# ToddThomson/Mila

Hardware: AMD Instinct MI355X
Metric: Gemma-4 12B decode tok/s (B=1, context 2048), 1xMI355X (higher is better)
Workload: dtype bf16; 1 GPU; Gemma-4 12B, weight policy bf16, B=1, prefill T=2048 then decode at positions 2048..; decode_mode=graph, replicas=1, parallelism=replicas only (no collective), bounded_local_kv=0

## Files before the change

mila_amd/csrc/attention.hip:

```cpp
#include "common.h"
#include "rms_common.h"
#include "rope_common.h"
#include "internal.h"
#include "attention_generic.h"
#include "attention_tiles.h"
#include "attention_decode_mfma.h"
#include "attention_decode_plan.h"
#include "attention_decode_scalar.h"

namespace mila {

__global__ __launch_bounds__(256) void kv_write_bf16_kernel(uint16_t* __restrict__ Kc, uint16_t* __restrict__ Vc,
                                                            const uint16_t* __restrict__ k,
                                                            const uint16_t* __restrict__ v, int64_t total_vec,
                                                            int chunk, int NKV, int HS, int start_pos, int capacity)
{
    const int hv = HS / 8;
    const int64_t stride = (int64_t)gridDim.x * 256;
    for (int64_t i = (int64_t)blockIdx.x * 256 + threadIdx.x; i < total_vec; i += stride)
    {
        const int e = (int)(i % hv);
        int64_t r = i / hv;
        const int n = (int)(r % NKV);
        r /= NKV;
        const int t = (int)(r % chunk);
        const int b = (int)(r / chunk);
        const int row = (start_pos + t) % capacity;
        const size_t dst = ((((size_t)b * NKV + n) * capacity + row) * hv + e) * 8;
        st16(Kc + dst, ld16(k + i * 8));
        st16(Vc + dst, ld16(v + i * 8));
    }
}

struct AttnParams
{
    uint16_t* Y;
    const uint16_t* Q;
    int64_t q_b_stride;
    uint16_t* K;
    uint16_t* V;
    float* scratch;
    int no_combine;
    const uint8_t* warm_a; int64_t warm_a_lines; int warm_a_blocks;
    const uint8_t* warm_b; int64_t warm_b_lines; int warm_b_blocks; int64_t warm_b_pair;
    uint32_t* tickets;
    int NH, NKV, capacity, position, window, splits;
    float scale;
    const int32_t* pos_dev;
    int flat;
    int64_t raw_b_stride;
    const uint16_t* q_raw;
    const uint16_t* k_raw;
    const uint16_t* v_raw;
    const uint16_t* qw;
    const uint16_t* kw;
    const uint16_t* vw;
    const float* cos_cache;
    const float* sin_cache;
    float eps;
    int pos_stride;
};

template <int HS>
__device__ __forceinline__ void head_row_post(const uint16_t* __restrict__ src, const uint16_t* __restrict__ w, bool rotate,
                                              const float* cos_row, const float* sin_row, float eps,
                                              uint16_t* dst_lds, uint16_t* dst_glb)
{
    constexpr int hv = HS / 16;
    const int lane = threadIdx.x & 63;
    const bool act = lane < hv;
    const int l2 = act ? lane : 0;
    const u32x4 xlo = ld16(src + (size_t)l2 * 8), xhi = ld16(src + (size_t)(l2 + hv) * 8);
    u32x4 wlo = u32x4{0u, 0u, 0u, 0u}, whi = wlo;
    if (w) { wlo = ld16(w + (size_t)l2 * 8); whi = ld16(w + (size_t)(l2 + hv) * 8); }
    const float rstd = rms_rstd_wave(src, HS, eps);
    if (act)
    {
        u32x4 lo, hi;
        if (w) { lo = rms_apply8(xlo, wlo, rstd, 0.0f); hi = rms_apply8(xhi, whi, rstd, 0.0f); }
        else { lo = rms_apply8_now(xlo, rstd); hi = rms_apply8_now(xhi, rstd); }
        if (rotate) rope_rotate8_vals(lo, hi, cos_row, sin_row, lane * 8);
        if (dst_lds) { st16(dst_lds + (size_t)lane * 8, lo); st16(dst_lds + (size_t)(lane + hv) * 8, hi); }
        if (dst_glb) { st16(dst_glb + (size_t)lane * 8, lo); st16(dst_glb + (size_t)(lane + hv) * 8, hi); }
    }
}

template <bool SC1>
__device__ __forceinline__ float partial_ld(const float* p)
{
    if constexpr (SC1)
        return __hip_atomic_load((const __attribute__((address_space(1))) float*)p, __ATOMIC_RELAXED, __HIP_MEMORY_SCOPE_AGENT);
    else
        return *p;
}
template <bool SC1>
__device__ __forceinline__ uint16_t combine_dim(const float* __restrict__ base, int HS, int splits, int d)
{
    const int STR = HS + 4;
    const int s = threadIdx.x & 63;
    float vals[16];
#pragma unroll
    for (int u = 0; u < 16; ++u) vals[u] = (u < splits) ? partial_ld<SC1>(base + (size_t)u * STR + d) : 0.0f;
    const float ms = (s < splits) ? partial_ld<SC1>(base + (size_t)s * STR + HS) : -INFINITY;
    const float ls = (s < splits) ? partial_ld<SC1>(base + (size_t)s * STR + HS + 1) : 0.0f;
    float acc = 0.0f;
    const float M = wave_max(ms);
    const float fs = (ms == -INFINITY) ? 0.0f : __expf(ms - M);
    const float L = wave_sum(ls * fs);
    const int n8 = (splits + 7) & ~7;
    for (int i0 = 0; i0 < n8; i0 += 16)
    {
        if (i0 > 0)
        {
#pragma unroll
            for (int u = 0; u < 16; ++u) vals[u] = (i0 + u < splits) ? partial_ld<SC1>(base + (size_t)(i0 + u) * STR + d) : 0.0f;
        }
#pragma unroll
        for (int u = 0; u < 16; ++u)
        {
            const float f = __uint_as_float(__builtin_amdgcn_readlane(__float_as_uint(fs), min(i0 + u, 63)));
            if (i0 + u < n8) acc = fmaf(vals[u], f, acc);
        }
    }
    return f32_to_bf16_bits(L > 0.0f ? acc / L : 0.0f);
}

__device__ __forceinline__ void warm_lines(const uint8_t* __restrict__ base, int64_t nlines, int64_t tid, int64_t nthreads, float* never,
                                           int64_t pair = 0)
{
    uint32_t acc = 0;
    int64_t i = tid;
    auto at = [&](int64_t l) { return pair ? base + (l & 1) * pair + (l >> 1) * 128 : base + l * 128; };
    for (; i + 7 * nthreads < nlines; i += 8 * nthreads)
    {
        uint32_t v[8];
#pragma unroll
        for (int u = 0; u < 8; ++u) v[u] = *reinterpret_cast<const uint32_t*>(at(i + u * nthreads));
#pragma unroll
        for (int u = 0; u < 8; ++u) acc ^= v[u];
    }
    for (; i < nlines; i += nthreads) acc ^= *reinterpret_cast<const uint32_t*>(at(i));
    if (acc == 0x12345679u && never != nullptr) never[0] = 1.0f;
}

#ifdef MILA_ATTN_STAMPS
__device__ unsigned long long g_attn_stamps[2];
#endif

#define MILA_ATTN_LEAD_PARAMS const int32_t* pos_dev, uint16_t* K, uint16_t* V, const uint16_t* q_raw, int NH, int NKV, int capacity, int window, int splits, int flat
#define MILA_ATTN_LEAD_ARGS(p) (p).pos_dev, (p).K, (p).V, (p).q_raw, (p).NH, (p).NKV, (p).capacity, (p).window, (p).splits, ((p).flat | ((p).pos_stride ? 2 : 0))
__device__ __forceinline__ AttnParams attn_params(MILA_ATTN_LEAD_PARAMS, const AttnParams& tail)
{
    AttnParams p = tail;
    p.pos_dev = pos_dev; p.K = K; p.V = V; p.q_raw = q_raw;
    p.NH = NH; p.NKV = NKV; p.capacity = capacity; p.window = window; p.splits = splits; p.flat = flat & 1; p.pos_stride = (flat >> 1) & 1;
    return p;
}

template <int HS, int GH, bool FUSED>
__global__ __launch_bounds__(kDecodeWaves * 64) void attn_decode_kernel(MILA_ATTN_LEAD_PARAMS, const AttnParams tail)
{
#ifdef MILA_ATTN_STAMPS
    const unsigned long long entry_ = __builtin_amdgcn_s_memtime();
#endif
    const AttnParams p = attn_params(pos_dev, K, V, q_raw, NH, NKV, capacity, window, splits, flat, tail);
    using Row = DecodeGeomBf16<HS>;
    constexpr int NW = kDecodeWaves, EPL = Row::EPL, NPAIR = Row::NPAIR, ACTIVE = Row::ACTIVE, PG = Row::PG, STR = HS + 2;
    extern __shared__ __attribute__((aligned(16))) unsigned char smem_raw[];
    float* sm = reinterpret_cast<float*>(smem_raw);
    uint16_t* qs = reinterpret_cast<uint16_t*>(smem_raw + (size_t)NW * GH * STR * sizeof(float));

    const int lane = threadIdx.x & 63, wave = threadIdx.x >> 6;
    const bool owner = lane < ACTIVE;
    const int GS = p.NH / p.NKV, hgroups = GS / GH;
    if (!p.flat && (int)blockIdx.x >= p.splits)
    {
        const int64_t wb = ((int64_t)(blockIdx.x - p.splits) * gridDim.y + blockIdx.y) * gridDim.z + blockIdx.z;
        warm_lines(p.warm_a, p.warm_a_lines, wb * (NW * 64) + threadIdx.x, (int64_t)p.warm_a_blocks * gridDim.y * gridDim.z * (NW * 64),
                   p.scratch);
        return;
    }
    const int ngrp = p.NKV * hgroups;
    const int split = p.flat ? (int)blockIdx.x / ngrp : (int)blockIdx.x, grp = p.flat ? (int)blockIdx.x % ngrp : (int)blockIdx.y;
    const int kvh = grp / hgroups, hg = grp % hgroups;
    const int h0 = kvh * GS + hg * GH;
    const int b = blockIdx.z;
    const int pos = p.pos_dev ? p.pos_dev[b * p.pos_stride] : p.position;
    const int len = pos + 1;
    const int band_begin = (p.window > 0) ? max(0, len - p.window) : 0;
    const int band = len - band_begin;
    const int chunk = (band + p.splits - 1) / p.splits;
    const int begin = band_begin + split * chunk;
    const int end = min(begin + chunk, len);
    const bool owns_new = FUSED && pos >= begin && pos < end;

    uint16_t* kbase = p.K + ((size_t)b * p.NKV + kvh) * p.capacity * HS;
    uint16_t* vbase = p.V + ((size_t)b * p.NKV + kvh) * p.capacity * HS;

    struct KVG { uint32_t k[PG][NPAIR], v[PG][NPAIR]; };
    auto load_group = [&](KVG& gbuf, int base) {
#pragma unroll
        for (int j = 0; j < PG; ++j)
        {
            const int pp = base + NW * j;
            if (owner && pp < end && !(FUSED && pp == pos))
            {
                const size_t r = (size_t)(pp % p.capacity) * HS + lane * EPL;
                load_row<EPL>(gbuf.k[j], kbase + r);
                load_row<EPL>(gbuf.v[j], vbase + r);
            }
            else
            {
#pragma unroll
                for (int e = 0; e < NPAIR; ++e) { gbuf.k[j][e] = 0u; gbuf.v[j][e] = 0u; }
            }
        }
    };

    int base = begin + wave;
    KVG ga, gb;
    if (base < end) load_group(ga, base);
#ifdef MILA_ATTN_STAMPS
    if (blockIdx.x == 0 && blockIdx.y == 0 && blockIdx.z == 0 && threadIdx.x == 0)
    {
        g_attn_stamps[0] += __builtin_amdgcn_s_memtime() - entry_;
        g_attn_stamps[1] += 1;
    }
#endif

    uint32_t q[GH][NPAIR];
    if constexpr (FUSED)
    {
        const int half = HS / 2;
        const float* cos_row = p.cos_cache + (size_t)pos * half;
        const float* sin_row = p.sin_cache + (size_t)pos * half;
        const int nrows = GH + (owns_new ? 2 : 0);
        for (int r = wave; r < nrows; r += NW)
        {
            if (r < GH)
                head_row_post<HS>(p.q_raw + (size_t)b * p.raw_b_stride + (size_t)(h0 + r) * HS, p.qw, true, cos_row, sin_row, p.eps, qs + (size_t)r * HS, nullptr);
            else if (r == GH)
                head_row_post<HS>(p.k_raw + (size_t)b * p.raw_b_stride + (size_t)kvh * HS, p.kw, true, cos_row, sin_row, p.eps, qs + (size_t)GH * HS,
                                  (hg == 0) ? kbase + (size_t)(pos % p.capacity) * HS : nullptr);
            else
                head_row_post<HS>(p.v_raw + (size_t)b * p.raw_b_stride + (size_t)kvh * HS, p.vw, false, cos_row, sin_row, p.eps, qs + (size_t)(GH + 1) * HS,
                                  (hg == 0) ? vbase + (size_t)(pos % p.capacity) * HS : nullptr);
        }
        __syncthreads();
#pragma unroll
        for (int g = 0; g < GH; ++g)
        {
            if (owner) load_row<EPL>(q[g], qs + (size_t)g * HS + lane * EPL);
            else
            {
#pragma unroll
                for (int e = 0; e < NPAIR; ++e) q[g][e] = 0u;
            }
        }
    }
    else
    {
#pragma unroll
        for (int g = 0; g < GH; ++g)
        {
            const uint16_t* qp = p.Q + (size_t)b * (p.q_b_stride ? (size_t)p.q_b_stride : (size_t)p.NH * HS) + (size_t)(h0 + g) * HS + lane * EPL;
            if (owner) load_row<EPL>(q[g], qp);
            else
            {
#pragma unroll
                for (int e = 0; e < NPAIR; ++e) q[g][e] = 0u;
            }
        }
    }

    float m[GH], l[GH], o[GH][EPL];
#pragma unroll
    for (int g = 0; g < GH; ++g)
    {
        m[g] = -INFINITY;
        l[g] = 0.0f;
#pragma unroll
        for (int e = 0; e < EPL; ++e) o[g][e] = 0.0f;
    }

    auto patch_new = [&](KVG& gbuf, int base_) {
        if constexpr (FUSED)
        {
            if (owns_new)
            {
#pragma unroll
                for (int j = 0; j < PG; ++j)
                    if (base_ + NW * j == pos && owner)
                    {
                        load_row<EPL>(gbuf.k[j], qs + (size_t)GH * HS + lane * EPL);
                        load_row<EPL>(gbuf.v[j], qs + (size_t)(GH + 1) * HS + lane * EPL);
                    }
            }
        }
    };
    auto compute_group = [&](const KVG& gbuf, int base_) {
        float sc[PG][GH];
#pragma unroll
        for (int j = 0; j < PG; ++j)
#pragma unroll
            for (int g = 0; g < GH; ++g)
            {
                float a = 0.0f;
#pragma unroll
                for (int e = 0; e < NPAIR; ++e) a = dot2_bf16(as_bf16x2(q[g][e]), as_bf16x2(gbuf.k[j][e]), a);
                sc[j][g] = a;
            }
        decode_softmax_step<GH, Row>(sc, gbuf.v, m, l, o, base_, end, p.scale);
    };
    for (;;)
    {
        if (base >= end) break;
        int nb = base + NW * PG;
        if (nb < end) load_group(gb, nb);
        patch_new(ga, base);
        compute_group(ga, base);
        base = nb;
        if (base >= end) break;
        nb = base + NW * PG;
        if (nb < end) load_group(ga, nb);
        patch_new(gb, base);
        compute_group(gb, base);
        base = nb;
    }

    const DecodeFinishArgs a{p.Y, p.scratch, p.NH, p.splits, split, b, h0, p.tickets != nullptr};
    decode_finish<HS, GH, Row>(a, m, l, o, sm);
    if (p.splits > 1 && p.tickets != nullptr)
    {
        __shared__ int s_last;
        __syncthreads();
        uint32_t* tk = p.tickets + (size_t)b * gridDim.y + blockIdx.y;
        if (threadIdx.x == 0)
        {
            const uint32_t t = __hip_atomic_fetch_add(tk, 1u, __ATOMIC_ACQ_REL, __HIP_MEMORY_SCOPE_AGENT);
            const int last = (t == (uint32_t)(p.splits - 1));
            if (last) __hip_atomic_store(tk, 0u, __ATOMIC_RELAXED, __HIP_MEMORY_SCOPE_AGENT);
            s_last = last;
        }
        __syncthreads();
        if (s_last)
        {
            for (int idx = threadIdx.x; idx < GH * HS; idx += NW * 64)
            {
                const int g = idx / HS, d = idx % HS;
                const int h = h0 + g;
                const float* base = p.scratch + ((size_t)b * p.NH + h) * p.splits * (HS + 4);
                p.Y[((size_t)b * p.NH + h) * HS + d] = combine_dim<true>(base, HS, p.splits, d);
            }
        }
    }
}

__global__ __launch_bounds__(64) void attn_combine_kernel(uint16_t* __restrict__ Y, const float* __restrict__ scratch, int NH,
                                                          int HS, int splits, const uint8_t* __restrict__ warm, int64_t warm_lines_n, int64_t warm_pair, int flat_gh)
{
    int h = blockIdx.x, zc = blockIdx.z;
    const int b = blockIdx.y;
    if (flat_gh > 0)
    {
        const int ngroups = NH / flat_gh, grp = (int)blockIdx.x % ngroups, r = (int)blockIdx.x / ngroups;
        h = grp * flat_gh + r % flat_gh;
        zc = r / flat_gh;
    }
    else if ((int)blockIdx.z >= HS / 64)
    {
        const int64_t wb = ((int64_t)(blockIdx.z - HS / 64) * gridDim.y + blockIdx.y) * gridDim.x + blockIdx.x;
        warm_lines(warm, warm_lines_n, wb * 64 + threadIdx.x, (int64_t)(gridDim.z - HS / 64) * gridDim.y * gridDim.x * 64, nullptr, warm_pair);
        return;
    }
    const int d = zc * 64 + threadIdx.x;
    const float* base = scratch + ((size_t)b * NH + h) * splits * (HS + 4);
    Y[((size_t)b * NH + h) * HS + d] = combine_dim<false>(base, HS, splits, d);
}


template <int HS>
__global__ __launch_bounds__(256) void attn_decode_mfma_kernel(MILA_ATTN_LEAD_PARAMS, const AttnParams tail)
{
    extern __shared__ __attribute__((aligned(16))) unsigned char smem_mfma[];
    const AttnParams p = attn_params(pos_dev, K, V, q_raw, NH, NKV, capacity, window, splits, flat, tail);
    const int pos = p.pos_dev ? p.pos_dev[(int)blockIdx.z * p.pos_stride] : p.position;
    const MfmaDecodeArgs a{p.Q, p.q_b_stride, p.scratch, p.NH, p.NKV, p.capacity, pos + 1, p.window, p.splits, p.scale};
    attn_decode_mfma_body<HS>(a, MfmaStageBf16<HS>{p.K, p.V}, smem_mfma);
}

__global__ __launch_bounds__(256) void attn_combine_many_kernel(uint16_t* __restrict__ Y, const float* __restrict__ scratch, int NH, int HS, int splits)
{
    __shared__ float s_acc[4][64], s_m[4], s_l[4];
    const int h = blockIdx.x, b = blockIdx.y, lane = threadIdx.x & 63, wave = threadIdx.x >> 6;
    const int d = blockIdx.z * 64 + lane;
    const int STR = HS + 4;
    const int s0 = wave * 64, n = min(64, splits - s0);
    const float* base = scratch + (((size_t)b * NH + h) * splits + s0) * STR;
    float acc = 0.0f, M = -INFINITY, L = 0.0f;
    if (n > 0)
    {
        float vals[16];
#pragma unroll
        for (int u = 0; u < 16; ++u) vals[u] = (u < n) ? base[(size_t)u * STR + d] : 0.0f;
        const float ms = (lane < n) ? base[(size_t)lane * STR + HS] : -INFINITY;
        const float ls = (lane < n) ? base[(size_t)lane * STR + HS + 1] : 0.0f;
        M = wave_max(ms);
        const float fs = (ms == -INFINITY) ? 0.0f : __expf(ms - M);
        L = wave_sum(ls * fs);
        const int n16 = (n + 15) & ~15;
        for (int i0 = 0; i0 < n16; i0 += 16)
        {
            if (i0 > 0)
            {
#pragma unroll
                for (int u = 0; u < 16; ++u) vals[u] = (i0 + u < n) ? base[(size_t)(i0 + u) * STR + d] : 0.0f;
            }
#pragma unroll
            for (int u = 0; u < 16; ++u)
            {
                const float f = __uint_as_float(__builtin_amdgcn_readlane(__float_as_uint(fs), min(i0 + u, 63)));
                acc = fmaf(vals[u], f, acc);
            }
        }
    }
    s_acc[wave][lane] = acc;
    if (lane == 0) { s_m[wave] = M; s_l[wave] = L; }
    __syncthreads();
    if (wave == 0)
    {
        float Mt = fmaxf(fmaxf(s_m[0], s_m[1]), fmaxf(s_m[2], s_m[3]));
        float Lt = 0.0f, out = 0.0f;
#pragma unroll
        for (int w = 0; w < 4; ++w)
        {
            const float f = (s_m[w] == -INFINITY) ? 0.0f : __expf(s_m[w] - Mt);
            Lt = fmaf(s_l[w], f, Lt);
            out = fmaf(s_acc[w][lane], f, out);
        }
        Y[((size_t)b * NH + h) * HS + d] = f32_to_bf16_bits(Lt > 0.0f ? out / Lt : 0.0f);
    }
}

enum DecodeForm { DF_SCALAR, DF_MFMA, DF_GENERIC };
struct DecodePlan
{
    DecodeForm form;
    int splits, band_max;
    int gh, hgroups;
    int flat;
    bool prologue;
    size_t partial_floats;
    size_t scratch_need;
};

constexpr int kMaxSplits = 64;
constexpr int kMaxSplitsMfma = 256;
static int g_tune_positions_per_split = 64;
MILA_TUNE("attn.positions_per_split", g_tune_positions_per_split);
static int g_attn_max_wgs = 256;
MILA_TUNE("attn.max_workgroups", g_attn_max_wgs);
static int g_attn_gh512 = 2;
MILA_TUNE("attn.heads_per_group_512", g_attn_gh512);
static int g_tune_decode_mfma = 1;
MILA_TUNE("attn.mfma_decode", g_tune_decode_mfma);
static int g_tune_kvfp8_mfma = 1;
MILA_TUNE("attn.kvfp8_mfma_decode", g_tune_kvfp8_mfma);
static int g_mfma_min_band = 8192;
MILA_TUNE("attn.mfma_min_band", g_mfma_min_band);
static int g_attn_xcd_local = 0;
MILA_TUNE("attn.xcd_local", g_attn_xcd_local);

static int band_bucket(int len, int capacity)
{
    int b = 4096;
    while (b < len && b < capacity) b <<= 1;
    return min(b, capacity);
}
static int heads_per_group(int GS, int HS) { return HS >= 512 ? (GS >= g_attn_gh512 && g_attn_gh512 == 4 ? 4 : (GS >= 2 ? 2 : 1)) : (GS >= 4 ? 4 : GS); }
static int decode_splits(int B, int NKV, int hgroups, int band)
{
    const int cap = max(1, g_attn_max_wgs / (NKV * hgroups * B));
    const int pps = g_tune_positions_per_split >= 8 ? g_tune_positions_per_split : 64;
    return max(1, min(min((band + pps - 1) / pps, cap), kMaxSplits));
}
static bool mfma_decode_applies(int NH, int NKV, int HS, int band_max)
{
    return g_tune_decode_mfma && HS == 512 && NKV > 0 && (NH / NKV) % 16 == 0 && band_max >= g_mfma_min_band;
}
static int mfma_decode_splits(int B, int NH, int NKV, int band_max)
{
    const int groups = NKV * ((NH / NKV) / 16) * B;
    const int s = (band_max + 127) / 128;
    return max(1, min(min(s, max(1, kNumCU / groups)), kMaxSplitsMfma));
}
static size_t decode_scratch_bytes(int B, int NH, int HS, int splits, bool q_rows)
{
    return (size_t)B * NH * splits * (HS + 4) * sizeof(float) + (q_rows ? (size_t)B * NH * HS * 2 : 0);
}

static DecodePlan plan_decode(int B, int NH, int NKV, int HS, int capacity, int window, int len_hint, bool fused, bool hooks, bool kvfp8 = false)
{
    const bool scalar_only = kvfp8 && !g_tune_kvfp8_mfma;
    DecodePlan d{};
    const int GS = NH / NKV;
    const bool split_kernel = decode_scalar_head_size(HS);
    d.band_max = (window > 0 && window < capacity) ? window : (len_hint > 0 ? band_bucket(len_hint, capacity) : capacity);
    d.gh = heads_per_group(GS, HS);
    d.hgroups = GS / d.gh;
    if (mfma_decode_applies(NH, NKV, HS, d.band_max) && !hooks && !scalar_only)
    {
        d.form = DF_MFMA;
        d.splits = mfma_decode_splits(B, NH, NKV, d.band_max);
        d.prologue = fused;
    }
    else
    {
        d.form = split_kernel ? DF_SCALAR : DF_GENERIC;
        d.splits = decode_splits(B, NKV, d.hgroups, d.band_max);
        d.flat = (g_attn_xcd_local && split_kernel && (NKV * d.hgroups) % 8 == 0 && !hooks) ? 1 : 0;
    }
    d.partial_floats = (size_t)B * NH * d.splits * (HS + 4);
    d.scratch_need = (d.form == DF_MFMA || (d.form == DF_SCALAR && d.splits > 1)) ? decode_scratch_bytes(B, NH, HS, d.splits, d.prologue) : 0;
    return d;
}
int launch_attn_combine_many(uint16_t* Y, const float* partials, int B, int NH, int HS, int splits, hipStream_t s)
{
    hipLaunchKernelGGL(attn_combine_many_kernel, dim3(NH, B, HS / 64), dim3(256), 0, s, Y, partials, NH, HS, splits);
    return check_hip(hipGetLastError(), "attn_combine_many");
}
static int launch_decode_mfma(const AttnParams& p, int B, hipStream_t s)
{
    constexpr int HS = 512;
    note_form("attn_decode_mfma");
    static bool attr_set = false;
    const size_t lds = mfma_decode_lds_bytes<HS>();
    if (!attr_set)
    {
        int rc = check_hip(hipFuncSetAttribute(reinterpret_cast<const void*>(attn_decode_mfma_kernel<HS>), hipFuncAttributeMaxDynamicSharedMemorySize, (int)lds), "hipFuncSetAttribute(attn_decode_mfma)");
        if (rc) return rc;
        attr_set = true;
    }
    const int n16 = (p.NH / p.NKV) / 16;
    hipLaunchKernelGGL((attn_decode_mfma_kernel<HS>), dim3(p.splits, p.NKV * n16, B), dim3(256), lds, s, MILA_ATTN_LEAD_ARGS(p), p);
    int rc = check_hip(hipGetLastError(), "attn_decode_mfma");
    if (rc) return rc;
    return launch_attn_combine_many(p.Y, p.scratch, B, p.NH, HS, p.splits, s);
}

template <int HS, int GH, bool FUSED>
static int launch_decode(const AttnParams& p, int B, hipStream_t s)
{
    const int hgroups = (p.NH / p.NKV) / GH;
    note_form("attn_decode");
    const size_t lds = (size_t)kDecodeWaves * GH * (HS + 2) * sizeof(float) + (size_t)(GH + 2) * HS * 2;
    const int wa = (p.warm_a && p.warm_a_lines > 0) ? p.warm_a_blocks : 0;
    if (p.flat)
    {
        hipLaunchKernelGGL((attn_decode_kernel<HS, GH, FUSED>), dim3(p.NKV * hgroups * p.splits, 1, B), dim3(kDecodeWaves * 64), lds, s, MILA_ATTN_LEAD_ARGS(p), p);
        int rc = check_hip(hipGetLastError(), "attn_decode (xcd-local)");
        if (rc || p.splits <= 1) return rc;
        hipLaunchKernelGGL(attn_combine_kernel, dim3(p.NH * (HS / 64), B, 1), dim3(64), 0, s, p.Y, p.scratch, p.NH, HS, p.splits, nullptr, 0, 0, GH);
        return check_hip(hipGetLastError(), "attn_combine (xcd-local)");
    }
    hipLaunchKernelGGL((attn_decode_kernel<HS, GH, FUSED>), dim3(p.splits + wa, p.NKV * hgroups, B), dim3(kDecodeWaves * 64), lds, s, MILA_ATTN_LEAD_ARGS(p), p);
    int rc = check_hip(hipGetLastError(), "attn_decode");
    if (rc) return rc;
    if (p.splits > 1 && !p.no_combine && !p.tickets)
    {
        const int wbk = (p.warm_b && p.warm_b_lines > 0) ? p.warm_b_blocks : 0;
        hipLaunchKernelGGL(attn_combine_kernel, dim3(p.NH, B, HS / 64 + wbk), dim3(64), 0, s, p.Y, p.scratch, p.NH, HS, p.splits, p.warm_b,
                           p.warm_b_lines, p.warm_b_pair, 0);
        rc = check_hip(hipGetLastError(), "attn_combine");
    }
    return rc;
}

template <bool FUSED>
static int dispatch_hs(int HS, int gh, const AttnParams& p, int B, hipStream_t s)
{
    if (decode_scalar_head_size(HS))
    {
        const int GS = p.NH / p.NKV;
        if (!decode_group_size_ok(GS)) return set_error(MILA_E_UNSUPPORTED, "attention: group size %d (NH/NKV) must be 1,2,4,8,16 or 32", GS);
        const int rc = dispatch_decode_scalar<true>(HS, gh, [&](auto hs, auto g) { return launch_decode<decltype(hs)::value, decltype(g)::value, FUSED>(p, B, s); });
        if (rc == kNoDecodeKernel) return set_error(MILA_E_UNSUPPORTED, "attention: no kernel for %d heads per workgroup at HS=%d", gh, HS);
        return rc;
    }
    if constexpr (!FUSED)
    {
        if (p.pos_dev) return set_error(MILA_E_UNSUPPORTED, "attention: the device-position form needs a head size of 64, 128, 256 or 512 (got %d)", HS);
        const int64_t qbs = p.q_b_stride ? p.q_b_stride : (int64_t)p.NH * HS;
        GenericAttnParams g{p.Y, p.Q, p.K, p.V, qbs, qbs, (int64_t)p.NKV * p.capacity * HS, (int64_t)p.capacity * HS, HS,
                            B, 1, p.NH, p.NKV, HS, p.capacity, p.position, p.window, p.scale};
        return launch_attn_generic(g, s);
    }
    return set_error(MILA_E_UNSUPPORTED, "attention: head size %d must be 64, 128, 256 or 512", HS);
}

static int run_decode(const DecodePlan& d, AttnParams p, int B, int HS, size_t scratch_bytes, const char* who, hipStream_t stream)
{
    const bool fused = p.q_raw != nullptr;
    p.splits = d.splits;
    p.flat = d.flat;
    if (d.scratch_need && (!p.scratch || scratch_bytes < d.scratch_need))
        return set_error(MILA_E_SCRATCH_TOO_SMALL, "%s: scratch %zu bytes < required %zu", who, scratch_bytes, d.scratch_need);
    if (d.form != DF_MFMA) return fused ? dispatch_hs<true>(HS, d.gh, p, B, stream) : dispatch_hs<false>(HS, d.gh, p, B, stream);
    if (d.prologue)
    {
        uint16_t* q_tmp = reinterpret_cast<uint16_t*>(p.scratch + d.partial_floats);
        for (int b = 0; b < B; ++b)
        {
            uint16_t* kc = p.K + (size_t)b * p.NKV * p.capacity * HS;
            uint16_t* vc = p.V + (size_t)b * p.NKV * p.capacity * HS;
            const size_t ro = (size_t)b * p.raw_b_stride;
            const int rc = p.pos_dev ? mila_cdna4_fused_qkv_post_devpos(q_tmp + (size_t)b * p.NH * HS, kc, vc, p.q_raw + ro, p.k_raw + ro, p.v_raw + ro, p.qw, p.kw, p.vw, p.cos_cache,
                                                                        p.sin_cache, p.NH, p.NKV, HS, p.pos_dev + (size_t)b * p.pos_stride, p.capacity, p.eps,
                                                                        reinterpret_cast<mila_stream_t>(stream))
                                     : mila_cdna4_fused_qkv_post(q_tmp + (size_t)b * p.NH * HS, kc, vc, p.q_raw + ro, p.k_raw + ro, p.v_raw + ro, p.qw, p.kw, p.vw, p.cos_cache,
                                                                 p.sin_cache, p.NH, p.NKV, HS, p.position, p.capacity, p.eps, reinterpret_cast<mila_stream_t>(stream));
            if (rc) return rc;
        }
        p.Q = q_tmp;
        p.q_b_stride = 0;
    }
    return launch_decode_mfma(p, B, stream);
}

static int unfused_decode(const char* who, uint16_t* Y, const uint16_t* Q, int64_t q_b_stride, const uint16_t* Kc, const uint16_t* Vc, void* scratch, size_t scratch_bytes, int B,
                          int NH, int NKV, int HS, int capacity, int position, const int32_t* pos_dev, int len_hint, int window, float scale, hipStream_t stream)
{
    AttnParams p{};
    p.Y = Y; p.Q = Q; p.q_b_stride = q_b_stride; p.K = const_cast<uint16_t*>(Kc); p.V = const_cast<uint16_t*>(Vc); p.scratch = reinterpret_cast<float*>(scratch);
    p.NH = NH; p.NKV = NKV; p.capacity = capacity; p.position = position; p.pos_dev = pos_dev; p.window = window; p.scale = scale;
    return run_decode(plan_decode(B, NH, NKV, HS, capacity, window, len_hint, false, false), p, B, HS, scratch_bytes, who, stream);
}

enum { FD_BATCH = 1, FD_TICKETS = 2, FD_PARTIALS = 4, FD_ROWS = 8 };
static int fused_decode(const char* who, const mila_fused_attn_args& a, int B, int64_t raw_b_stride, int flags, hipStream_t stream)
{
    MILA_REQUIRE((a.Y || (flags & FD_PARTIALS)) && a.Kc && a.Vc && a.q_raw && a.k_raw && a.v_raw && a.qw && a.kw && a.cos_cache && a.sin_cache &&
                 (a.tickets || !(flags & FD_TICKETS)), "%s: null pointer", who);
    if (flags & FD_BATCH)
    {
        MILA_REQUIRE(B > 0 && a.NH > 0 && a.NKV > 0 && a.NH % a.NKV == 0, "%s: bad sizes (B=%d NH=%d NKV=%d)", who, B, a.NH, a.NKV);
        MILA_REQUIRE(B == 1 || raw_b_stride >= (int64_t)a.NKV * a.HS, "%s: raw_b_stride %lld is shorter than a K row", who, (long long)raw_b_stride);
    }
    else
        MILA_REQUIRE(a.NH > 0 && a.NKV > 0 && a.NH % a.NKV == 0, "%s: bad head counts (NH=%d NKV=%d)", who, a.NH, a.NKV);
    MILA_REQUIRE(a.capacity > 0 && a.window >= 0 && (a.position_dev || a.position >= 0), "%s: bad sizes", who);
    MILA_REQUIRE(a.HS % 16 == 0, "%s: HS=%d must be a multiple of 16", who, a.HS);
    MILA_REQUIRE(a.warm_a_blocks >= 0 && a.warm_a_blocks <= 64 && a.warm_b_blocks >= 0 && a.warm_b_blocks <= 64, "%s: warm block counts must be in [0, 64]", who);
    if (a.tickets)
        MILA_REQUIRE(a.ticket_count >= mila_cdna4_attn_decode_ticket_count(1, a.NH), "%s: %zu tickets < required %zu", who, a.ticket_count,
                     mila_cdna4_attn_decode_ticket_count(1, a.NH));
    AttnParams p{};
    p.Y = a.Y; p.K = a.Kc; p.V = a.Vc; p.scratch = reinterpret_cast<float*>(a.scratch);
    p.NH = a.NH; p.NKV = a.NKV; p.capacity = a.capacity; p.position = a.position; p.pos_dev = a.position_dev; p.window = a.window; p.scale = a.scale;
    p.q_raw = a.q_raw; p.k_raw = a.k_raw; p.v_raw = a.v_raw; p.raw_b_stride = raw_b_stride; p.qw = a.qw; p.kw = a.kw; p.vw = a.vw;
    p.cos_cache = a.cos_cache; p.sin_cache = a.sin_cache; p.eps = a.eps;
    p.tickets = a.tickets;
    p.no_combine = (flags & FD_PARTIALS) ? 1 : 0;
    p.pos_stride = (flags & FD_ROWS) ? 1 : 0;
    if (a.warm_a && a.warm_a_bytes >= 128 && a.warm_a_blocks > 0) { p.warm_a = (const uint8_t*)a.warm_a; p.warm_a_lines = (int64_t)(a.warm_a_bytes / 128); p.warm_a_blocks = a.warm_a_blocks; }
    if (a.warm_b && a.warm_b_bytes >= 128 && a.warm_b_blocks > 0) { p.warm_b = (const uint8_t*)a.warm_b; p.warm_b_lines = (int64_t)(a.warm_b_bytes / 128); p.warm_b_blocks = a.warm_b_blocks; p.warm_b_pair = (int64_t)a.warm_b_pair_offset; }
    DecodePlan d = plan_decode((flags & FD_ROWS) ? 1 : B, a.NH, a.NKV, a.HS, a.capacity, a.window, a.position_dev ? a.position : a.position + 1, true,
                               p.tickets || p.no_combine || p.warm_a || p.warm_b);
    if ((flags & FD_ROWS) && B > 1)
    {
        d.partial_floats *= (size_t)B;
        if (d.scratch_need) d.scratch_need = decode_scratch_bytes(B, a.NH, a.HS, d.splits, d.prologue);
    }
    if (flags & FD_PARTIALS) MILA_REQUIRE(d.splits > 1, "%s: this (window, capacity) runs unsplit; use fused_attn_decode_bf16", who);
    if (!a.position_dev)
    {
        const int band = live_band(a.position + 1, a.window);
        MILA_REQUIRE(band <= a.capacity, "%s: live band %d exceeds the cache capacity %d", who, band, a.capacity);
    }
    return run_decode(d, p, B, a.HS, a.scratch_bytes, who, stream);
}
static mila_fused_attn_args fused_args(uint16_t* Y, uint16_t* Kc, uint16_t* Vc, const uint16_t* q_raw, const uint16_t* k_raw, const uint16_t* v_raw, const uint16_t* qw,
                                       const uint16_t* kw, const uint16_t* vw, const float* cos_cache, const float* sin_cache, void* scratch, size_t scratch_bytes,
                                       uint32_t* tickets, size_t ticket_count, int NH, int NKV, int HS, int capacity, int position, const int32_t* position_dev, int window,
                                       float scale, float eps)
{
    return mila_fused_attn_args{Y, Kc, Vc, q_raw, k_raw, v_raw, qw, kw, vw, cos_cache, sin_cache, scratch, scratch_bytes, tickets, ticket_count, nullptr, 0, 0, nullptr, 0, 0, 0,
                                NH, NKV, HS, capacity, position, position_dev, window, scale, eps};
}

KvFp8DecodeShape plan_decode_kvfp8(int B, int NH, int NKV, int HS, int capacity, int window, int len_hint)
{
    const DecodePlan d = plan_decode(B, NH, NKV, HS, capacity, window, len_hint, false, false, true);
    return KvFp8DecodeShape{d.form == DF_MFMA, d.splits, d.gh, d.hgroups, d.scratch_need};
}
int launch_attn_combine(uint16_t* Y, const float* partials, int B, int NH, int HS, int splits, hipStream_t s)
{
    hipLaunchKernelGGL(attn_combine_kernel, dim3(NH, B, HS / 64), dim3(64), 0, s, Y, partials, NH, HS, splits, nullptr, 0, 0, 0);
    return check_hip(hipGetLastError(), "attn_combine");
}

__global__ __launch_bounds__(256) void mha_kv_write_kernel(uint16_t* __restrict__ Kc, uint16_t* __restrict__ Vc, const uint16_t* __restrict__ QKV,
                                                           int64_t total, int T, int C, int HS, int start_pos, int capacity)
{
    const int NH = C / HS;
    const int64_t stride = (int64_t)gridDim.x * 256;
    for (int64_t i = (int64_t)blockIdx.x * 256 + threadIdx.x; i < total; i += stride)
    {
        const int c = (int)(i % C);
        const int64_t bt = i / C;
        const int t = (int)(bt % T), b = (int)(bt / T);
        const int h = c / HS, d = c - h * HS;
        const size_t dst = (((size_t)b * NH + h) * capacity + (start_pos + t)) * HS + d;
        const uint16_t* row = QKV + bt * 3 * (int64_t)C;
        Kc[dst] = row[C + c];
        Vc[dst] = row[2 * C + c];
    }
}
__global__ __launch_bounds__(256) void mha_kv_write_vec_kernel(uint16_t* __restrict__ Kc, uint16_t* __restrict__ Vc, const uint16_t* __restrict__ QKV,
                                                               int64_t total_vec, int T, int C, int HS, int start_pos, int capacity)
{
    const int NH = C / HS, cv = C / 8;
    const int64_t stride = (int64_t)gridDim.x * 256;
    for (int64_t i = (int64_t)blockIdx.x * 256 + threadIdx.x; i < total_vec; i += stride)
    {
        const int c = (int)(i % cv) * 8;
        const int64_t bt = i / cv;
        const int t = (int)(bt % T), b = (int)(bt / T);
        const int h = c / HS, d = c - h * HS;
        const size_t dst = (((size_t)b * NH + h) * capacity + (start_pos + t)) * HS + d;
        const uint16_t* row = QKV + bt * 3 * (int64_t)C;
        st16(Kc + dst, ld16(row + C + c));
        st16(Vc + dst, ld16(row + 2 * C + c));
    }
}

}

using namespace mila;

extern "C" {

#ifdef MILA_ATTN_STAMPS
MILA_API int mila_dbg_attn_stamps(unsigned long long* out2)
{
    return (int)hipMemcpyFromSymbol(out2, HIP_SYMBOL(mila::g_attn_stamps), 2 * sizeof(unsigned long long));
}
#endif

int mila_cdna4_kv_write_bf16(uint16_t* Kc, uint16_t* Vc, const uint16_t* k, const uint16_t* v, int B, int chunk, int NKV,
                             int HS, int start_pos, int capacity, mila_stream_t stream)
{
    MILA_REQUIRE(Kc && Vc && k && v, "kv_write_bf16: null pointer");
    MILA_REQUIRE(B > 0 && chunk > 0 && NKV > 0 && HS > 0 && capacity > 0, "kv_write_bf16: bad sizes");
    MILA_REQUIRE(HS % 8 == 0, "kv_write_bf16: HS=%d must be a multiple of 8", HS);
    MILA_REQUIRE(start_pos >= 0, "kv_write_bf16: negative start position");
    MILA_REQUIRE(chunk <= capacity, "kv_write_bf16: chunk %d exceeds the cache capacity %d", chunk, capacity);
    const int64_t total_vec = (int64_t)B * chunk * NKV * (HS / 8);
    int blocks = ceil_div(total_vec, 256);
    if (blocks > 2048) blocks = 2048;
    hipLaunchKernelGGL(kv_write_bf16_kernel, dim3(blocks), dim3(256), 0, as_stream(stream), Kc, Vc, k, v, total_vec, chunk,
                       NKV, HS, start_pos, capacity);
    MILA_LAUNCH_CHECK("kv_write_bf16");
}

size_t mila_cdna4_attn_decode_scratch_bytes(int B, int NH, int HS)
{
    if (B <= 0 || NH <= 0 || HS <= 0) return 0;
    return std::max(decode_scratch_bytes(B, NH, HS, kMaxSplits, false), HS == 512 ? decode_scratch_bytes(B, NH, HS, kMaxSplitsMfma, true) : 0);
}

int mila_cdna4_attn_decode_band_bucket(int len, int capacity) { return capacity > 0 ? band_bucket(len, capacity) : 0; }

int mila_cdna4_attn_decode_bf16(uint16_t* Y, const uint16_t* Q, const uint16_t* Kc, const uint16_t* Vc, void* scratch,
                                size_t scratch_bytes, int B, int NH, int NKV, int HS, int capacity, int len, int window,
                                float scale, mila_stream_t stream)
{
    MILA_REQUIRE(Y && Q && Kc && Vc, "attn_decode_bf16: null pointer");
    MILA_REQUIRE(B > 0 && NH > 0 && NKV > 0 && NH % NKV == 0, "attn_decode_bf16: bad head counts (NH=%d NKV=%d)", NH, NKV);
    MILA_REQUIRE(len > 0 && capacity > 0, "attn_decode_bf16: len and capacity must be positive (len=%d capacity=%d)", len, capacity);
    MILA_REQUIRE(window >= 0, "attn_decode_bf16: negative window");
    const int band = live_band(len, window);
    MILA_REQUIRE(band <= capacity, "attn_decode_bf16: live band %d exceeds the cache capacity %d", band, capacity);
    return unfused_decode("attn_decode_bf16", Y, Q, 0, Kc, Vc, scratch, scratch_bytes, B, NH, NKV, HS, capacity, len - 1, nullptr, len, window, scale, as_stream(stream));
}

int mila_cdna4_attn_decode_bf16_devpos(uint16_t* Y, const uint16_t* Q, const uint16_t* Kc, const uint16_t* Vc, void* scratch,
                                       size_t scratch_bytes, int B, int NH, int NKV, int HS, int capacity,
                                       const int32_t* position_dev, int max_len, int window, float scale,
                                       mila_stream_t stream)
{
    MILA_REQUIRE(Y && Q && Kc && Vc && position_dev, "attn_decode_bf16_devpos: null pointer");
    MILA_REQUIRE(B > 0 && NH > 0 && NKV > 0 && NH % NKV == 0, "attn_decode_bf16_devpos: bad head counts (NH=%d NKV=%d)", NH, NKV);
    MILA_REQUIRE(max_len > 0 && capacity > 0 && window >= 0, "attn_decode_bf16_devpos: bad sizes");
    const int band = live_band(max_len, window);
    MILA_REQUIRE(band <= capacity, "attn_decode_bf16_devpos: live band %d exceeds the cache capacity %d", band, capacity);
    return unfused_decode("attn_decode_bf16_devpos", Y, Q, 0, Kc, Vc, scratch, scratch_bytes, B, NH, NKV, HS, capacity, 0, position_dev, max_len, window, scale, as_stream(stream));
}

int mila_cdna4_fused_attn_decode_bf16(uint16_t* Y, uint16_t* Kc, uint16_t* Vc, const uint16_t* q_raw, const uint16_t* k_raw,
                                      const uint16_t* v_raw, const uint16_t* qw, const uint16_t* kw, const uint16_t* vw,
                                      const float* cos_cache, const float* sin_cache, void* scratch, size_t scratch_bytes,
                                      int NH, int NKV, int HS, int capacity, int position, const int32_t* position_dev,
                                      int window, float scale, float eps, mila_stream_t stream)
{
    return fused_decode("fused_attn_decode_bf16", fused_args(Y, Kc, Vc, q_raw, k_raw, v_raw, qw, kw, vw, cos_cache, sin_cache, scratch, scratch_bytes, nullptr, 0, NH, NKV, HS,
                                                             capacity, position, position_dev, window, scale, eps), 1, 0, 0, as_stream(stream));
}

int mila_cdna4_fused_attn_decode_batch_bf16(uint16_t* Y, uint16_t* Kc, uint16_t* Vc, const uint16_t* q_raw, const uint16_t* k_raw,
                                            const uint16_t* v_raw, int64_t raw_b_stride, const uint16_t* qw, const uint16_t* kw, const uint16_t* vw,
                                            const float* cos_cache, const float* sin_cache, void* scratch, size_t scratch_bytes, int B,
                                            int NH, int NKV, int HS, int capacity, int position, const int32_t* position_dev,
                                            int window, float scale, float eps, mila_stream_t stream)
{
    return fused_decode("fused_attn_decode_batch_bf16", fused_args(Y, Kc, Vc, q_raw, k_raw, v_raw, qw, kw, vw, cos_cache, sin_cache, scratch, scratch_bytes, nullptr, 0, NH, NKV,
                                                                   HS, capacity, position, position_dev, window, scale, eps), B, raw_b_stride, FD_BATCH, as_stream(stream));
}
int mila_cdna4_fused_attn_decode_rows_bf16(uint16_t* Y, uint16_t* Kc, uint16_t* Vc, const uint16_t* q_raw, const uint16_t* k_raw, const uint16_t* v_raw, int64_t raw_b_stride,
                                           const uint16_t* qw, const uint16_t* kw, const uint16_t* vw, const float* cos_cache, const float* sin_cache, void* scratch,
                                           size_t scratch_bytes, int B, int NH, int NKV, int HS, int capacity, const int32_t* positions_dev, int max_len, int window, float scale,
                                           float eps, mila_stream_t stream)
{
    MILA_REQUIRE(positions_dev != nullptr, "fused_attn_decode_rows_bf16: positions_dev is required (the rows' positions live on the device)");
    MILA_REQUIRE(max_len >= 0 && max_len <= capacity, "fused_attn_decode_rows_bf16: max_len %d outside 0 .. the capacity %d", max_len, capacity);
    MILA_REQUIRE(decode_scalar_head_size(HS), "fused_attn_decode_rows_bf16: head size %d must be 64, 128, 256 or 512", HS);
    return fused_decode("fused_attn_decode_rows_bf16", fused_args(Y, Kc, Vc, q_raw, k_raw, v_raw, qw, kw, vw, cos_cache, sin_cache, scratch, scratch_bytes, nullptr, 0, NH, NKV,
                                                                  HS, capacity, max_len, positions_dev, window, scale, eps),
                        B, raw_b_stride, FD_BATCH | FD_ROWS, as_stream(stream));
}

int mila_cdna4_mha_kv_write_bf16(uint16_t* Kc, uint16_t* Vc, const uint16_t* QKV, int B, int T, int C, int NH, int start_pos, int capacity,
                                 mila_stream_t stream)
{
    MILA_REQUIRE(Kc && Vc && QKV, "mha_kv_write_bf16: null pointer");
    MILA_REQUIRE(B > 0 && T > 0 && C > 0 && NH > 0 && C % NH == 0 && capacity > 0, "mha_kv_write_bf16: bad sizes (B=%d T=%d C=%d NH=%d capacity=%d)", B, T, C, NH, capacity);
    MILA_REQUIRE(start_pos >= 0 && start_pos + T <= capacity, "mha_kv_write_bf16: positions [%d, %d) do not fit the cache capacity %d", start_pos, start_pos + T, capacity);
    const int HS = C / NH;
    const bool vec = HS % 8 == 0 && ((uintptr_t)QKV % 16 == 0) && ((uintptr_t)Kc % 16 == 0) && ((uintptr_t)Vc % 16 == 0);
    const int64_t total = vec ? (int64_t)B * T * (C / 8) : (int64_t)B * T * C;
    int blocks = ceil_div(total, 256);
    if (blocks > 4096) blocks = 4096;
    if (vec) hipLaunchKernelGGL(mha_kv_write_vec_kernel, dim3(blocks), dim3(256), 0, as_stream(stream), Kc, Vc, QKV, total, T, C, HS, start_pos, capacity);
    else hipLaunchKernelGGL(mha_kv_write_kernel, dim3(blocks), dim3(256), 0, as_stream(stream), Kc, Vc, QKV, total, T, C, HS, start_pos, capacity);
    MILA_LAUNCH_CHECK("mha_kv_write_bf16");
}

size_t mila_cdna4_mha_decode_scratch_bytes(int B, int C, int NH)
{
    if (B <= 0 || C <= 0 || NH <= 0 || C % NH != 0) return 0;
    return mila_cdna4_attn_decode_scratch_bytes(B, NH, C / NH);
}

int mila_cdna4_mha_decode_bf16(uint16_t* Y, const uint16_t* QKV, uint16_t* Kc, uint16_t* Vc, void* scratch, size_t scratch_bytes, int B, int C,
                               int NH, int capacity, int position, mila_stream_t stream)
{
    MILA_REQUIRE(Y && QKV && Kc && Vc, "mha_decode_bf16: null pointer");
    MILA_REQUIRE(B > 0 && C > 0 && NH > 0 && C % NH == 0 && capacity > 0, "mha_decode_bf16: bad sizes (B=%d C=%d NH=%d capacity=%d)", B, C, NH, capacity);
    MILA_REQUIRE(position >= 0 && position < capacity, "mha_decode_bf16: position %d out of range [0, %d)", position, capacity);
    const int HS = C / NH;
    int rc = mila_cdna4_mha_kv_write_bf16(Kc, Vc, QKV, B, 1, C, NH, position, capacity, stream);
    if (rc) return rc;
    return unfused_decode("mha_decode_bf16", Y, QKV, 3 * (int64_t)C, Kc, Vc, scratch, scratch_bytes, B, NH, NH, HS, capacity, position, nullptr, 0, 0, 1.0f / sqrtf((float)HS),
                          as_stream(stream));
}

int mila_cdna4_attn_decode_split_count(int B, int NH, int NKV, int HS, int capacity, int window, int len_hint)
{
    if (B <= 0 || NH <= 0 || NKV <= 0 || NH % NKV != 0 || capacity <= 0 || window < 0) return 0;
    return plan_decode(B, NH, NKV, HS, capacity, window, len_hint, true, true).splits;
}

int mila_cdna4_fused_attn_decode_partials_bf16(uint16_t* Kc, uint16_t* Vc, const uint16_t* q_raw, const uint16_t* k_raw,
                                               const uint16_t* v_raw, const uint16_t* qw, const uint16_t* kw, const uint16_t* vw,
                                               const float* cos_cache, const float* sin_cache, void* scratch, size_t scratch_bytes,
                                               int NH, int NKV, int HS, int capacity, int position, const int32_t* position_dev,
                                               int window, float scale, float eps, mila_stream_t stream)
{
    return fused_decode("fused_attn_decode_partials_bf16", fused_args(nullptr, Kc, Vc, q_raw, k_raw, v_raw, qw, kw, vw, cos_cache, sin_cache, scratch, scratch_bytes, nullptr, 0,
                                                                      NH, NKV, HS, capacity, position, position_dev, window, scale, eps), 1, 0, FD_PARTIALS, as_stream(stream));
}

size_t mila_cdna4_attn_decode_ticket_count(int B, int NH)
{
    if (B <= 0 || NH <= 0) return 0;
    return (size_t)B * NH;
}

int mila_cdna4_fused_attn_decode_onepass_bf16(uint16_t* Y, uint16_t* Kc, uint16_t* Vc, const uint16_t* q_raw, const uint16_t* k_raw,
                                              const uint16_t* v_raw, const uint16_t* qw, const uint16_t* kw, const uint16_t* vw,
                                              const float* cos_cache, const float* sin_cache, void* scratch, size_t scratch_bytes,
                                              uint32_t* tickets, size_t ticket_count, int NH, int NKV, int HS, int capacity, int position,
                                              const int32_t* position_dev, int window, float scale, float eps, mila_stream_t stream)
{
    return fused_decode("fused_attn_decode_onepass_bf16", fused_args(Y, Kc, Vc, q_raw, k_raw, v_raw, qw, kw, vw, cos_cache, sin_cache, scratch, scratch_bytes, tickets, ticket_count,
                                                                     NH, NKV, HS, capacity, position, position_dev, window, scale, eps), 1, 0, FD_TICKETS, as_stream(stream));
}

int mila_cdna4_fused_attn_decode_ex(const mila_fused_attn_args* a, mila_stream_t stream)
// ... 27 lines not shown
```

Before: 225.7 tok/s.

## Overlap decode attention prologue with early KV loads and cheaper index math

Reworks the fused decode attention kernel so the KV-cache group loads start before the Q/K/V RMS-norm and RoPE prologue finishes. Each wave now handles one prologue row, and the rotation and LDS store are deferred until after the loads are issued. It also reads the position word early and replaces integer division and modulo with a host-computed magic multiplier, power-of-two shifts and an incremental ring-row counter. KV loads become branchless with masking, and small page groups get a second group prefetched up front. The aim is to shorten kernel latency in the prologue, at the cost of more registers and an assumption that heads per KV group is a power of two.

After: 228.5 tok/s, median of 6. 1.3% higher.

```diff
diff --git a/mila_amd/csrc/attention.hip b/mila_amd/csrc/attention.hip
--- a/mila_amd/csrc/attention.hip
+++ b/mila_amd/csrc/attention.hip
@@ -7,6 +7,7 @@
 #include "attention_decode_mfma.h"
 #include "attention_decode_plan.h"
 #include "attention_decode_scalar.h"
+#include "split_div.h"
 
 namespace mila {
 
@@ -59,31 +60,8 @@
     const float* sin_cache;
     float eps;
     int pos_stride;
+    uint32_t split_mul, split_shift;
 };
-
-template <int HS>
-__device__ __forceinline__ void head_row_post(const uint16_t* __restrict__ src, const uint16_t* __restrict__ w, bool rotate,
-                                              const float* cos_row, const float* sin_row, float eps,
-                                              uint16_t* dst_lds, uint16_t* dst_glb)
-{
-    constexpr int hv = HS / 16;
-    const int lane = threadIdx.x & 63;
-    const bool act = lane < hv;
-    const int l2 = act ? lane : 0;
-    const u32x4 xlo = ld16(src + (size_t)l2 * 8), xhi = ld16(src + (size_t)(l2 + hv) * 8);
-    u32x4 wlo = u32x4{0u, 0u, 0u, 0u}, whi = wlo;
-    if (w) { wlo = ld16(w + (size_t)l2 * 8); whi = ld16(w + (size_t)(l2 + hv) * 8); }
-    const float rstd = rms_rstd_wave(src, HS, eps);
-    if (act)
-    {
-        u32x4 lo, hi;
-        if (w) { lo = rms_apply8(xlo, wlo, rstd, 0.0f); hi = rms_apply8(xhi, whi, rstd, 0.0f); }
-        else { lo = rms_apply8_now(xlo, rstd); hi = rms_apply8_now(xhi, rstd); }
-        if (rotate) rope_rotate8_vals(lo, hi, cos_row, sin_row, lane * 8);
-        if (dst_lds) { st16(dst_lds + (size_t)lane * 8, lo); st16(dst_lds + (size_t)(lane + hv) * 8, hi); }
-        if (dst_glb) { st16(dst_glb + (size_t)lane * 8, lo); st16(dst_glb + (size_t)(lane + hv) * 8, hi); }
-    }
-}
 
 template <bool SC1>
 __device__ __forceinline__ float partial_ld(const float* p)
@@ -144,7 +122,7 @@
 }
 
 #ifdef MILA_ATTN_STAMPS
-__device__ unsigned long long g_attn_stamps[2];
+__device__ unsigned long long g_attn_stamps[3];
 #endif
 
 #define MILA_ATTN_LEAD_PARAMS const int32_t* pos_dev, uint16_t* K, uint16_t* V, const uint16_t* q_raw, int NH, int NKV, int capacity, int window, int splits, int flat
@@ -163,16 +141,26 @@
 #ifdef MILA_ATTN_STAMPS
     const unsigned long long entry_ = __builtin_amdgcn_s_memtime();
 #endif
-    const AttnParams p = attn_params(pos_dev, K, V, q_raw, NH, NKV, capacity, window, splits, flat, tail);
     using Row = DecodeGeomBf16<HS>;
     constexpr int NW = kDecodeWaves, EPL = Row::EPL, NPAIR = Row::NPAIR, ACTIVE = Row::ACTIVE, PG = Row::PG, STR = HS + 2;
+    constexpr int GH_LOG2 = GH == 4 ? 2 : (GH == 2 ? 1 : 0);
+    constexpr bool PRE2 = PG < 8;
+    static_assert(GH == 1 || GH == 2 || GH == 4, "heads per workgroup: 1, 2 or 4");
+    static_assert(GH + 2 <= NW, "one prologue row per wave");
+    const int lane = threadIdx.x & 63, wave = __builtin_amdgcn_readfirstlane(threadIdx.x >> 6);
+    const bool owner = lane < ACTIVE;
+    const int b = blockIdx.z;
+
+    int lane_zero;
+    asm volatile("v_mov_b32 %0, 0" : "=v"(lane_zero));
+    const int32_t* pos_at = pos_dev ? pos_dev + b * ((flat >> 1) & 1) : reinterpret_cast<const int32_t*>(K);
+    const int pos_word = pos_at[lane_zero];
+
+    const AttnParams p = attn_params(pos_dev, K, V, q_raw, NH, NKV, capacity, window, splits, flat, tail);
     extern __shared__ __attribute__((aligned(16))) unsigned char smem_raw[];
     float* sm = reinterpret_cast<float*>(smem_raw);
     uint16_t* qs = reinterpret_cast<uint16_t*>(smem_raw + (size_t)NW * GH * STR * sizeof(float));
 
-    const int lane = threadIdx.x & 63, wave = threadIdx.x >> 6;
-    const bool owner = lane < ACTIVE;
-    const int GS = p.NH / p.NKV, hgroups = GS / GH;
     if (!p.flat && (int)blockIdx.x >= p.splits)
     {
         const int64_t wb = ((int64_t)(blockIdx.x - p.splits) * gridDim.y + blockIdx.y) * gridDim.z + blockIdx.z;
@@ -180,81 +168,41 @@
                    p.scratch);
         return;
     }
-    const int ngrp = p.NKV * hgroups;
-    const int split = p.flat ? (int)blockIdx.x / ngrp : (int)blockIdx.x, grp = p.flat ? (int)blockIdx.x % ngrp : (int)blockIdx.y;
-    const int kvh = grp / hgroups, hg = grp % hgroups;
-    const int h0 = kvh * GS + hg * GH;
-    const int b = blockIdx.z;
-    const int pos = p.pos_dev ? p.pos_dev[b * p.pos_stride] : p.position;
-    const int len = pos + 1;
-    const int band_begin = (p.window > 0) ? max(0, len - p.window) : 0;
-    const int band = len - band_begin;
-    const int chunk = (band + p.splits - 1) / p.splits;
-    const int begin = band_begin + split * chunk;
-    const int end = min(begin + chunk, len);
-    const bool owns_new = FUSED && pos >= begin && pos < end;
-
+    const int gs_log2 = __builtin_clz((unsigned)p.NKV) - __builtin_clz((unsigned)p.NH), hg_log2 = gs_log2 - GH_LOG2;
+    int split = (int)blockIdx.x, grp = (int)blockIdx.y;
+    if (p.flat)
+    {
+        const int ngrp = p.NKV << hg_log2;
+        split = (int)blockIdx.x / ngrp;
+        grp = (int)blockIdx.x % ngrp;
+    }
+    const int kvh = grp >> hg_log2, hg = grp & ((1 << hg_log2) - 1);
+    const int h0 = grp * GH;
     uint16_t* kbase = p.K + ((size_t)b * p.NKV + kvh) * p.capacity * HS;
     uint16_t* vbase = p.V + ((size_t)b * p.NKV + kvh) * p.capacity * HS;
 
-    struct KVG { uint32_t k[PG][NPAIR], v[PG][NPAIR]; };
-    auto load_group = [&](KVG& gbuf, int base) {
-#pragma unroll
-        for (int j = 0; j < PG; ++j)
-        {
-            const int pp = base + NW * j;
-            if (owner && pp < end && !(FUSED && pp == pos))
+    constexpr int hv = HS / 16;
+    const bool act = lane < hv;
+    const int l2 = act ? lane : 0;
+    const bool has_row = FUSED && wave < GH + 2, rotates = FUSED && wave <= GH;
+    uint32_t q[GH][NPAIR];
+    u32x4 lo = u32x4{0u, 0u, 0u, 0u}, hi = lo;
+    if constexpr (FUSED)
+    {
+        if (has_row)
+        {
+            const uint16_t* src = (wave < GH ? p.q_raw + (size_t)(h0 + wave) * HS : (wave == GH ? p.k_raw : p.v_raw) + (size_t)kvh * HS) + (size_t)b * p.raw_b_stride;
+            const uint16_t* w = wave < GH ? p.qw : (wave == GH ? p.kw : p.vw);
+            const u32x4 xlo = ld16(src + (size_t)l2 * 8), xhi = ld16(src + (size_t)(l2 + hv) * 8);
+            u32x4 wlo = u32x4{0u, 0u, 0u, 0u}, whi = wlo;
+            if (w) { wlo = ld16(w + (size_t)l2 * 8); whi = ld16(w + (size_t)(l2 + hv) * 8); }
+            const float rstd = rms_rstd_wave(src, HS, p.eps);
+            if (w) { lo = rms_apply8(xlo, wlo, rstd, 0.0f); hi = rms_apply8(xhi, whi, rstd, 0.0f); }
+            else { lo = rms_apply8_now(xlo, rstd); hi = rms_apply8_now(xhi, rstd); }
+            if (wave == GH + 1 && act)
             {
-                const size_t r = (size_t)(pp % p.capacity) * HS + lane * EPL;
-                load_row<EPL>(gbuf.k[j], kbase + r);
-                load_row<EPL>(gbuf.v[j], vbase + r);
-            }
-            else
-            {
-#pragma unroll
-                for (int e = 0; e < NPAIR; ++e) { gbuf.k[j][e] = 0u; gbuf.v[j][e] = 0u; }
-            }
-        }
-    };
-
-    int base = begin + wave;
-    KVG ga, gb;
-    if (base < end) load_group(ga, base);
-#ifdef MILA_ATTN_STAMPS
-    if (blockIdx.x == 0 && blockIdx.y == 0 && blockIdx.z == 0 && threadIdx.x == 0)
-    {
-        g_attn_stamps[0] += __builtin_amdgcn_s_memtime() - entry_;
-        g_attn_stamps[1] += 1;
-    }
-#endif
-
-    uint32_t q[GH][NPAIR];
-    if constexpr (FUSED)
-    {
-        const int half = HS / 2;
-        const float* cos_row = p.cos_cache + (size_t)pos * half;
-        const float* sin_row = p.sin_cache + (size_t)pos * half;
-        const int nrows = GH + (owns_new ? 2 : 0);
-        for (int r = wave; r < nrows; r += NW)
-        {
-            if (r < GH)
-                head_row_post<HS>(p.q_raw + (size_t)b * p.raw_b_stride + (size_t)(h0 + r) * HS, p.qw, true, cos_row, sin_row, p.eps, qs + (size_t)r * HS, nullptr);
-            else if (r == GH)
-                head_row_post<HS>(p.k_raw + (size_t)b * p.raw_b_stride + (size_t)kvh * HS, p.kw, true, cos_row, sin_row, p.eps, qs + (size_t)GH * HS,
-                                  (hg == 0) ? kbase + (size_t)(pos % p.capacity) * HS : nullptr);
-            else
-                head_row_post<HS>(p.v_raw + (size_t)b * p.raw_b_stride + (size_t)kvh * HS, p.vw, false, cos_row, sin_row, p.eps, qs + (size_t)(GH + 1) * HS,
-                                  (hg == 0) ? vbase + (size_t)(pos % p.capacity) * HS : nullptr);
-        }
-        __syncthreads();
-#pragma unroll
-        for (int g = 0; g < GH; ++g)
-        {
-            if (owner) load_row<EPL>(q[g], qs + (size_t)g * HS + lane * EPL);
-            else
-            {
-#pragma unroll
-                for (int e = 0; e < NPAIR; ++e) q[g][e] = 0u;
+                st16(qs + (size_t)(GH + 1) * HS + (size_t)lane * 8, lo);
+                st16(qs + (size_t)(GH + 1) * HS + (size_t)(lane + hv) * 8, hi);
             }
         }
     }
@@ -270,6 +218,98 @@
 #pragma unroll
                 for (int e = 0; e < NPAIR; ++e) q[g][e] = 0u;
             }
+        }
+    }
+
+    const uint32_t cap = (uint32_t)p.capacity;
+    const uint32_t row_step = cap >= (uint32_t)NW ? (uint32_t)NW : (uint32_t)NW % cap;
+
+    const int pos_read = __builtin_amdgcn_readfirstlane(pos_word);
+    const int pos = p.pos_dev ? pos_read : p.position;
+    const int len = pos + 1;
+    const int band_begin = (p.window > 0) ? max(0, len - p.window) : 0;
+    const int band = len - band_begin;
+    const int chunk = (int)split_div((uint32_t)(band + p.splits - 1), SplitDiv{p.split_mul, p.split_shift});
+    const int begin = band_begin + split * chunk;
+    const int end = min(begin + chunk, len);
+    const bool owns_new = FUSED && pos >= begin && pos < end;
+
+    const bool wrapped = (uint32_t)len > cap;
+    auto ring_row = [&](int pp) -> uint32_t {
+        if (!wrapped) return (uint32_t)pp;
+        return (cap & (cap - 1u)) == 0u ? (uint32_t)pp & (cap - 1u) : (uint32_t)pp % cap;
+    };
+    f32x4 c0 = f32x4{0.f, 0.f, 0.f, 0.f}, c1 = c0, s0 = c0, s1 = c0;
+    if constexpr (FUSED)
+    {
+        if (rotates)
+        {
+            const float* cos_row = p.cos_cache + (size_t)pos * (HS / 2) + l2 * 8;
+            const float* sin_row = p.sin_cache + (size_t)pos * (HS / 2) + l2 * 8;
+            c0 = *reinterpret_cast<const f32x4*>(cos_row); c1 = *reinterpret_cast<const f32x4*>(cos_row + 4);
+            s0 = *reinterpret_cast<const f32x4*>(sin_row); s1 = *reinterpret_cast<const f32x4*>(sin_row + 4);
+        }
+    }
+
+    struct KVG { uint32_t k[PG][NPAIR], v[PG][NPAIR]; };
+    int base = begin + wave;
+    uint32_t row = ring_row(base);
+    const uint32_t lane_el = owner ? (uint32_t)lane * EPL : 0u;
+    auto load_group = [&](KVG& gbuf, int base_) {
+#pragma unroll
+        for (int j = 0; j < PG; ++j)
+        {
+            const int pp = base_ + NW * j;
+            const bool valid = pp < end && !(FUSED && pp == pos);
+            const size_t r = (size_t)(valid ? row : 0u) * HS;
+            const uint32_t keep = (valid && owner) ? ~0u : 0u;
+            uint32_t kk[NPAIR], vv[NPAIR];
+            load_row<EPL>(kk, (kbase + r) + lane_el);
+            load_row<EPL>(vv, (vbase + r) + lane_el);
+            __builtin_amdgcn_sched_barrier(0);
+#pragma unroll
+            for (int e = 0; e < NPAIR; ++e) { gbuf.k[j][e] = kk[e] & keep; gbuf.v[j][e] = vv[e] & keep; }
+            row += row_step;
+            if (row >= cap) row -= cap;
+        }
+    };
+    KVG ga, gb;
+    load_group(ga, base);
+#ifdef MILA_ATTN_STAMPS
+    const bool stamps_ = blockIdx.x == 0 && blockIdx.y == 0 && blockIdx.z == 0 && threadIdx.x == 0;
+    bool stamp_score_ = true;
+    if (stamps_)
+    {
+        g_attn_stamps[0] += __builtin_amdgcn_s_memtime() - entry_;
+        g_attn_stamps[1] += 1;
+    }
+#endif
+    if constexpr (PRE2) load_group(gb, base + NW * PG);
+
+    if constexpr (FUSED)
+    {
+        if (rotates && act)
+        {
+            rope_rotate8_regs(lo, hi, c0, c1, s0, s1);
+            st16(qs + (size_t)wave * HS + (size_t)lane * 8, lo);
+            st16(qs + (size_t)wave * HS + (size_t)(lane + hv) * 8, hi);
+        }
+        __syncthreads();
+#pragma unroll
+        for (int g = 0; g < GH; ++g)
+        {
+            if (owner) load_row<EPL>(q[g], qs + (size_t)g * HS + lane * EPL);
+            else
+            {
+#pragma unroll
+                for (int e = 0; e < NPAIR; ++e) q[g][e] = 0u;
+            }
+        }
+        if (has_row && wave >= GH && owns_new && hg == 0 && act)
+        {
+            uint16_t* dst = (wave == GH ? kbase : vbase) + (size_t)ring_row(pos) * HS;
+            st16(dst + (size_t)lane * 8, lo);
+            st16(dst + (size_t)(lane + hv) * 8, hi);
         }
     }
 
@@ -310,23 +350,27 @@
                 for (int e = 0; e < NPAIR; ++e) a = dot2_bf16(as_bf16x2(q[g][e]), as_bf16x2(gbuf.k[j][e]), a);
                 sc[j][g] = a;
             }
+#ifdef MILA_ATTN_STAMPS
+        if (stamp_score_)
+        {
+            asm volatile("" :: "v"(sc[0][0]));
+            if (stamps_) g_attn_stamps[2] += __builtin_amdgcn_s_memtime() - entry_;
+            stamp_score_ = false;
+        }
+#endif
         decode_softmax_step<GH, Row>(sc, gbuf.v, m, l, o, base_, end, p.scale);
     };
-    for (;;)
-    {
-        if (base >= end) break;
-        int nb = base + NW * PG;
-        if (nb < end) load_group(gb, nb);
-        patch_new(ga, base);
-        compute_group(ga, base);
+    auto step = [&](KVG& cur, KVG& nxt, bool nxt_in_flight) -> bool {
+        if (base >= end) return false;
+        const int nb = base + NW * PG;
+        if (!nxt_in_flight && nb < end) load_group(nxt, nb);
+        patch_new(cur, base);
+        compute_group(cur, base);
         base = nb;
-        if (base >= end) break;
-        nb = base + NW * PG;
-        if (nb < end) load_group(ga, nb);
-        patch_new(gb, base);
-        compute_group(gb, base);
-        base = nb;
-    }
+        return true;
+    };
+    if (step(ga, gb, PRE2))
+        while (step(gb, ga, false) && step(ga, gb, false)) {}
 
     const DecodeFinishArgs a{p.Y, p.scratch, p.NH, p.splits, split, b, h0, p.tickets != nullptr};
     decode_finish<HS, GH, Row>(a, m, l, o, sm);
@@ -549,8 +593,12 @@
 }
 
 template <int HS, int GH, bool FUSED>
-static int launch_decode(const AttnParams& p, int B, hipStream_t s)
-{
+static int launch_decode(const AttnParams& params, int B, hipStream_t s)
+{
+    AttnParams p = params;
+    const SplitDiv sd = split_div_make((uint32_t)p.splits);
+    p.split_mul = sd.mul;
+    p.split_shift = sd.shift;
     const int hgroups = (p.NH / p.NKV) / GH;
     note_form("attn_decode");
     const size_t lds = (size_t)kDecodeWaves * GH * (HS + 2) * sizeof(float) + (size_t)(GH + 2) * HS * 2;
@@ -741,9 +789,9 @@
 extern "C" {
 
 #ifdef MILA_ATTN_STAMPS
-MILA_API int mila_dbg_attn_stamps(unsigned long long* out2)
-{
-    return (int)hipMemcpyFromSymbol(out2, HIP_SYMBOL(mila::g_attn_stamps), 2 * sizeof(unsigned long long));
+MILA_API int mila_dbg_attn_stamps(unsigned long long* out3)
+{
+    return (int)hipMemcpyFromSymbol(out3, HIP_SYMBOL(mila::g_attn_stamps), 3 * sizeof(unsigned long long));
 }
 #endif
 
diff --git a/mila_amd/csrc/split_div.h b/mila_amd/csrc/split_div.h
--- /dev/null
+++ b/mila_amd/csrc/split_div.h
@@ -0,0 +1,33 @@
+#pragma once
+#include <cstdint>
+
+#if defined(__HIPCC__) || defined(__CUDACC__)
+#define MILA_SPLIT_DIV_FN __host__ __device__ inline
+#else
+#define MILA_SPLIT_DIV_FN inline
+#endif
+
+namespace mila {
+
+struct SplitDiv
+{
+    uint32_t mul;
+    uint32_t shift;
+};
+
+MILA_SPLIT_DIV_FN SplitDiv split_div_make(uint32_t d)
+{
+    if (d <= 1u) return SplitDiv{0u, 0u};
+    uint32_t s = 0;
+    while ((2u << s) < d) ++s;
+    const uint64_t p = (uint64_t)1 << (32 + s);
+    return SplitDiv{(uint32_t)((p + d - 1) / d), s};
+}
+
+MILA_SPLIT_DIV_FN uint32_t split_div(uint32_t n, SplitDiv c)
+{
+    const uint32_t hi = (uint32_t)(((uint64_t)n * c.mul) >> 32);
+    return c.mul ? hi >> c.shift : n;
+}
+
+}
```
